# m-schuetz/SimLOD

Hardware: AMD Instinct MI355X
Metric: M points/sec inserted into octree (raster M samples/s @1080p under 'raster') (higher is better)
Workload: dtype f32+u32 (fp32 quantise/project, fp64 pixel coordinate, integer octree/atomics); 1 GPU; Morro Bay 36M stand-in (BASELINE config 2): 36000000 16 B points, fractal terrain, 36 x 1M ring batches resident in HBM, reset + 2.0 kernel_construct launches per step; raster 1920x1080; points_per_gpu=36000000, record_order=shuffled, parallelism=one global cube, level-3 cells dealt to 1 rank(s) by point count

## Files before the change

simlod_amd/csrc/construct.hip:

```cpp
#include <mutex>
#include "simlod_device.hpp"
#include "simlod_hip.h"
#include "simlod_internal.hpp"

namespace simlod {
namespace build {

#include "construct_state.inc"
#include "construct_begin.inc"
#include "construct_count.inc"
#include "construct_expand.inc"
#include "construct_voxelize.inc"
#include "construct_insert.inc"

static_assert(offsetof(Ctl, groupMax) == 44 && offsetof(Ctl, expandNs) + 4 * sizeof(uint64_t) == 184, "Ctl.groupMax at byte 44, Ctl.expandNs[4] at byte 184");

static inline uint64_t align_up(uint64_t v, uint64_t a) { return (v + a - 1) / a * a; }

static constexpr uint64_t ACCT_SPILL_FLOOR = 3500000;
bool layout_construct(BuildArgs& a, uint64_t capacity, bool coalesce, uint32_t groupLimit = SIMLOD_MAX_BATCHES_PER_LAUNCH, uint32_t exactGroup = 1) {
	a.dirCap = 2 * a.nodeCapacity + 65536;
	a.acct = exactGroup > 1u ? 1u : 0u;
	uint64_t off = 4096;
	a.offQueue = off;    off += align_up((uint64_t)CHUNK_QUEUE_CAPACITY * 8, 256);
	a.offSlots = off;    off += align_up((uint64_t)2 * SLOT_CAP * sizeof(SlotRec), 256);
	a.offHist = off;     off += align_up(((uint64_t)SLOT_CAP * HIST_BINS + HIST_EXTRA_WORDS) * 4, 256);
	a.offMap = off;      off += align_up((uint64_t)SLOT_CAP * HIST_BINS * 4, 256);
	a.offHistB = off;    off += align_up((uint64_t)(a.acct ? SLOT_CAP : 0u) * HIST_BINS * exactGroup * 4, 256);
	a.clearCap = 65536;
	a.offClear = off;    off += align_up((uint64_t)2 * a.clearCap * 8, 256);
	a.offTouched = off;  off += align_up((uint64_t)a.nodeCapacity * 4, 256);
	a.crossCap = 16384;
	a.offCross = off;    off += align_up((uint64_t)a.crossCap * 4, 256);
	a.offSplitTag = off; off += align_up((uint64_t)a.nodeCapacity * 8, 256);
	a.offRetryTag = off; off += align_up((uint64_t)a.nodeCapacity * 4, 256);
	a.offTouchTag = off; off += align_up((uint64_t)a.nodeCapacity * 4, 256);
	a.offStartOf = off;  off += align_up((uint64_t)a.nodeCapacity * 8, 256);
	a.offCntB = off;     off += align_up((uint64_t)(a.acct ? a.nodeCapacity : 0u) * exactGroup * 4, 256);
	a.hashCap = 1u << 17;
	a.offHashDir = off;  off += align_up((uint64_t)a.hashCap * sizeof(DirEntry), 256);
	a.offParent = off;   off += align_up((uint64_t)a.nodeCapacity * 4, 256);
	a.offNodeDir = off;  off += align_up((uint64_t)a.nodeCapacity * sizeof(NodeDir), 256);
	a.offChunkDir = off; off += align_up(2ull * a.dirCap * 8, 256);
	a.offLeafChunks = off; off += (uint64_t)a.nodeCapacity * LEAF_ROW_BYTES;
	a.offPaths = off; off += align_up((uint64_t)a.nodeCapacity * PATH_ROW * 8, 256);
	a.offTop = off;   off += align_up((uint64_t)TOP_CELLS * 4, 256);
	a.offKid = off;   off += align_up((uint64_t)a.nodeCapacity * 4, 256);
	a.voxItemCap = min(a.nodeCapacity + 2u * VOX_BIG_ITEMS, 1u << 20);
	a.offVoxItems = off; off += align_up(2ull * a.voxItemCap * sizeof(VoxItem), 256);
	const uint64_t perBatch = (uint64_t)SIMLOD_MAX_BATCH_SIZE * 4;
	const uint64_t fixedWork = ((uint64_t)SPILLING_CAPACITY + a.nodeCapacity / 8) * 32;
	a.groupMax = 1; a.groupCap = SIMLOD_MAX_BATCH_SIZE;
	if (capacity < off + 2 * perBatch + fixedWork + 4096 + 25ull * 65536) { a.spilledCap = 0; a.scratchBytes = off + 2 * perBatch + fixedWork; return false; }
	const uint64_t freeBytes = capacity - off - fixedWork - 4096;
	if (coalesce) a.groupMax = (uint32_t)std::max<uint64_t>(1, std::min<uint64_t>(std::min<uint32_t>(groupLimit, SIMLOD_MAX_BATCHES_PER_LAUNCH), freeBytes / (2 * perBatch + 20ull * SIMLOD_MAX_BATCH_SIZE)));
	if (a.acct) {
		if (freeBytes < 2ull * exactGroup * perBatch + 512 + ACCT_SPILL_FLOOR * 20032 / 1000) return false;
		a.groupMax = exactGroup;
	}
	a.groupCap = a.groupMax * SIMLOD_MAX_BATCH_SIZE;
	uint64_t cap = (freeBytes - 2ull * a.groupMax * perBatch - 512) * 1000 / (20 * 1000 + 32);
	if (cap > 0x7fffffffull - a.groupCap) cap = 0x7fffffffull - a.groupCap;
	a.spilledCap = (uint32_t)cap;
	a.workCap = a.spilledCap / SIMLOD_POINTS_PER_CHUNK + a.nodeCapacity / 8 + SPILLING_CAPACITY;
	a.offWork = off;     off += align_up((uint64_t)a.workCap * 32, 256);
	a.leafOfStride = align_up((uint64_t)a.groupCap * 4, 256) / 4;
	a.offLeafOf = off;   off += 2 * a.leafOfStride * 4 + align_up((uint64_t)a.spilledCap * 4, 256);
	a.offSpilled = off;  off += (uint64_t)a.spilledCap * 16;
	a.scratchBytes = off;
	return off <= capacity;
}

}
struct SideStream {
	hipStream_t stream;
	hipEvent_t expanded[SIMLOD_MAX_BATCHES_PER_LAUNCH], inserted[SIMLOD_MAX_BATCHES_PER_LAUNCH], tailDone;
	std::mutex enqueue;
};
void destroy_side_stream(SideStream* s) {
	(void)hipStreamSynchronize(s->stream);
	for (uint32_t i = 0; i < SIMLOD_MAX_BATCHES_PER_LAUNCH; i++) { (void)hipEventDestroy(s->expanded[i]); (void)hipEventDestroy(s->inserted[i]); }
	(void)hipEventDestroy(s->tailDone);
	(void)hipStreamDestroy(s->stream);
	delete s;
}
namespace build {
#ifndef SYNC_EVENT_FLAGS
#define SYNC_EVENT_FLAGS (hipEventDisableTiming | hipEventDisableSystemFence)
#endif
static SideStream* side_stream(Context& ctx) {
	int dev = 0;
	(void)hipGetDevice(&dev);
	if (dev < 0 || dev >= 64) return nullptr;
	std::lock_guard<std::mutex> hold(ctx.sideLock);
	if (ctx.side[dev] == nullptr) {
		SideStream* s = new SideStream();
		bool ok = hipStreamCreateWithFlags(&s->stream, hipStreamNonBlocking) == hipSuccess;
		const unsigned flags = ctx.tune(KNOB_EVENT_SYSTEM_FENCE, 0) != 0 ? (unsigned)hipEventDisableTiming : (unsigned)SYNC_EVENT_FLAGS;
		for (uint32_t i = 0; ok && i < SIMLOD_MAX_BATCHES_PER_LAUNCH; i++)
			ok = hipEventCreateWithFlags(&s->expanded[i], flags) == hipSuccess && hipEventCreateWithFlags(&s->inserted[i], flags) == hipSuccess;
		ok = ok && hipEventCreateWithFlags(&s->tailDone, flags) == hipSuccess;
		if (!ok) { (void)hipGetLastError(); delete s; return nullptr; }
		ctx.side[dev] = s;
	}
	return ctx.side[dev];
}

int launch_construct(Context& ctx, const SimlodUniforms* u, SimlodPoint* points, uint32_t* buffer, uint8_t* pers, SimlodNode* nodes,
                     SimlodStats* stats, uint64_t* frameStart, uint32_t* numBatchesUploaded, uint32_t* batchSizes, hipStream_t stream) {
	BuildArgs a{};
	a.ring = points; a.mom = reinterpret_cast<uint8_t*>(buffer); a.pers = pers; a.nodes = nodes; a.stats = stats;
	a.frameStart = frameStart; a.numBatchesUploaded = numBatchesUploaded; a.batchSizes = batchSizes;
	octree_box(u, a.size, a.minx, a.miny, a.minz);
	a.persCapacity = u->persistentBufferCapacity;
	a.frameCounter = u->frameCounter;
	a.nodeCapacity = ctx.nodeCapacity.load();
	a.trunkLo = ctx.trunkLo.load(); a.trunkHi = ctx.trunkHi.load();
	const bool coalesce = ctx.ingestMode.load() != 0u;
	uint32_t exactGroup = coalesce || ctx.tune(KNOB_DEBUG_BUDGET_US, 0) > 0 ? 1u : (uint32_t)std::min<int>(std::max(1, ctx.tune(KNOB_EXACT_GROUP, 5)), (int)ACCT_MAX_GROUP);
	if (exactGroup > 1u && SIMLOD_MEM_SAFETY_MARGIN + group_slack_bytes(2ull * SIMLOD_MAX_BATCH_SIZE, 0u) >= a.persCapacity) exactGroup = 1u;
	bool fits = false;
	for (; exactGroup > 1u && !fits; exactGroup -= fits ? 0u : 1u) fits = layout_construct(a, u->momentaryBufferCapacity, false, 1, exactGroup);
	if (!fits) fits = layout_construct(a, u->momentaryBufferCapacity, coalesce, (uint32_t)std::max(1, ctx.tune(KNOB_GROUP_BATCHES, 10)));
	if (fits && ((uint64_t)a.mom & (LEAF_ROW_BYTES - 1u)) == 0ull) {
		const Ctl* ctl = reinterpret_cast<const Ctl*>(a.mom);
		note_leaf_table(ctx, LeafTableRef{nodes, a.mom, a.mom + a.offLeafChunks, a.pers, &ctl->tableMagic, &ctl->tableBatch,
		                             &ctl->tableNodes, &ctl->tableSig, TABLE_MAGIC, LEAF_SLOTS, a.nodeCapacity});
	} else forget_leaf_table(ctx, nodes);
	const DeviceInfo& dev = device_info();

	note_upload_counter(numBatchesUploaded, 0u, false, true);
	const LaunchPlan plan = launch_plan(ctx, nodes, numBatchesUploaded);
	const uint32_t limit = plan.batches;
	const uint32_t take = a.acct != 0u && !plan.mayGroup ? 1u : a.groupMax;
	SIMLOD_LAUNCH(k_begin, dim3(fits ? dev.numCUs * 2 : 1u), dim3(TPB), stream, a, fits ? 0u : 1u, limit, ((uint32_t)ctx.tune(KNOB_DEBUG_FORCE_BARRIER_TIMEOUT, 0) & 1u) | (ctx.tune(KNOB_DEBUG_VOXELIZE_CLOCK, 0) != 0 ? 2u : 0u) | (plan.sideTablesStale ? 4u : 0u) | (ctx.tune(KNOB_DEBUG_IRREGULAR_CHILDREN, 0) != 0 ? 8u : 0u) | (((uint32_t)ctx.tune(KNOB_DEBUG_PHASE_WG, 0) & 0xffffu) << 8),
	              (uint32_t)std::max(0, ctx.tune(KNOB_DEBUG_BUDGET_US, 0)), take);
	if (fits) {
		const uint32_t gridPoints = dev.numCUs * (uint32_t)ctx.tune(KNOB_GRID_MULT, 8);
		const uint32_t numGroups = (limit + take - 1u) / take;
		const bool overlap = ctx.tune(KNOB_OVERLAP_TAIL, 1) != 0 && !profile_enabled() && numGroups > 1u;
		const bool single = take == 1u || limit <= 1u;
		const uint32_t expandWgs = (uint32_t)max(1, min(ctx.tune(KNOB_EXPAND_WGS, !single ? (int)dev.numCUs / 2 : (int)dev.numCUs / (overlap ? 4 : 2)), (int)dev.numCUs));
		SideStream* side = overlap ? side_stream(ctx) : nullptr;
		std::unique_lock<std::mutex> block;
		if (side != nullptr) block = std::unique_lock<std::mutex>(side->enqueue);
		const int countTpb = ctx.tune(KNOB_COUNT_TPB, 512);
		hipStream_t back = side != nullptr ? side->stream : stream;
		auto fail = [&](hipError_t e) { if (side != nullptr) (void)hipStreamSynchronize(side->stream); (void)hipGetLastError(); return (int)(e != hipSuccess ? e : hipErrorUnknown); };
		const uint32_t voxWgs = (uint32_t)max(1, ctx.tune(KNOB_VOXELIZE_WGS, (int)dev.numCUs * 2)) + VOXROOT_WGS;
		for (uint32_t b = 0; b < numGroups; b++) {
			if (single) {
				if (countTpb == 256) SIMLOD_LAUNCH((k_count<TPB, true>), dim3(gridPoints), dim3(TPB), stream, a, b);
				else SIMLOD_LAUNCH((k_count<512, true>), dim3(gridPoints / 2), dim3(512), stream, a, b);
			} else SIMLOD_LAUNCH((k_count<512, false>), dim3(gridPoints / 2), dim3(512), stream, a, b);
			SIMLOD_LAUNCH(k_queue, dim3(single ? 16 : 128), dim3(TPB), stream, a, b);
			if (side != nullptr && b > 0) { const hipError_t e = hipStreamWaitEvent(stream, side->inserted[b - 1], 0); if (e != hipSuccess) return fail(e); }
			SIMLOD_LAUNCH(k_hist, dim3(gridPoints), dim3(TPB), stream, a, b);
			if (!single) {
				SIMLOD_LAUNCH(k_expand<true>, dim3(expandWgs), dim3(ETPB), stream, a, b, 0u, 1u);
				SIMLOD_LAUNCH(k_hist2, dim3(gridPoints), dim3(TPB), stream, a, b);
			}
			const hipEvent_t expanded = side != nullptr ? side->expanded[b] : nullptr, inserted = side != nullptr ? side->inserted[b] : nullptr;
			const bool gated = expand_gate_enter(ctx, stream);
			SIMLOD_LAUNCH_STOP(k_expand<false>, dim3(expandWgs), dim3(ETPB), stream, expanded, a, b, single ? 0u : 1u, (uint32_t)SIMLOD_MAX_EXPAND_ROUNDS);
			expand_gate_leave(ctx, stream, expanded, gated);
			if (side != nullptr) { const hipError_t e = hipStreamWaitEvent(back, expanded, 0); if (e != hipSuccess) return fail(e); }
			if (!single && a.acct != 0u) SIMLOD_LAUNCH(k_rootpre, dim3(1), dim3(1024), back, a, b);
			if (single) SIMLOD_LAUNCH_STOP(k_insert<true>, dim3(gridPoints), dim3(TPB), back, inserted, a, b);
			else SIMLOD_LAUNCH_STOP(k_insert<false>, dim3(gridPoints), dim3(TPB), back, inserted, a, b);
			if (profile_dominant()) {
				hipEvent_t e0, e1;
				profile_kernel_events("k_voxelize", &e0, &e1);
				hipExtLaunchKernelGGL(k_voxelize, dim3(voxWgs), dim3(VTPB), 0, back, e0, e1, 0, a, b);
				{ const hipError_t e = hipGetLastError(); if (e != hipSuccess) return fail(e); }
			} else
			SIMLOD_LAUNCH(k_voxelize, dim3(voxWgs), dim3(VTPB), back, a, b);
		}
		if (side != nullptr) {
			hipError_t e = hipEventRecord(side->tailDone, back);
			if (e == hipSuccess) e = hipStreamWaitEvent(stream, side->tailDone, 0);
			if (e != hipSuccess) return fail(e);
		}
		const uint32_t gridNodes = (a.nodeCapacity + TPB - 1) / TPB;
		SIMLOD_LAUNCH(k_voxdone, dim3(min(gridNodes, dev.numCUs)), dim3(TPB), stream, a);
		SIMLOD_LAUNCH(k_stats, dim3(min(gridNodes, dev.numCUs)), dim3(TPB), stream, a);
	}
	SIMLOD_LAUNCH(k_finish, dim3(1), dim3(64), stream, a, fits ? 1u : 0u, plan.feedback, (const uint32_t*)numBatchesUploaded, plan.seq);
	if (profile_enabled()) profile_close(stream);
	hipError_t e = hipGetLastError();
	if (e != hipSuccess) return (int)e;
	return fits ? 0 : (int)hipErrorInvalidValue;
}

uint64_t construct_min_bytes(uint32_t nodeCapacity) {
	BuildArgs a{};
	a.nodeCapacity = nodeCapacity;
	layout_construct(a, 0, false);
	return a.scratchBytes + 4096 + 26ull * 65536;
}

}
}
```

simlod_amd/csrc/construct_expand.inc:

```

static constexpr uint32_t VTPB = 1024;
#ifndef VOX_SPT_N
#define VOX_SPT_N 8
#endif
static constexpr uint32_t VOX_SPT = VOX_SPT_N;
static constexpr uint32_t VOX_PIECE = VTPB * VOX_SPT;
static constexpr uint32_t VOX_BIG_ITEMS = 65536;
static constexpr uint32_t VOX_SMALL = 512;
static constexpr uint32_t VOX_SMALL_PIECE = 128;
static constexpr uint32_t LDS_LEVELS = 7;
static constexpr uint32_t CUBE_WORDS = 8192 + 1024 + 256 + 64 + 16 + 4 + 4;
struct VoxItem { uint32_t leaf, s0, s1, ptBase, ptFirst; };
__device__ __forceinline__ VoxItem* vox_items(const BuildArgs& a, const BatchCtl* bc) { return at<VoxItem>(a, a.offVoxItems) + (uint64_t)(bc->ordinal & 1u) * a.voxItemCap; }

#ifndef ALLOC_WAVES_N
#define ALLOC_WAVES_N 10
#endif
static constexpr uint32_t ALLOC_WAVES = ALLOC_WAVES_N, ALLOC_LEAVES = 64 * ALLOC_WAVES;
struct AllocRec {
	uint32_t node, existing, additional, fromPool;
	uint32_t dirNew, prefix;
	unsigned long long firstIdx, mem;
	SimlodChunk* head; SimlodChunk* tail;
};
// ... 65 lines not shown
		dirBase = (uint32_t)__shfl((int)dirBase, 0, 64); itemBase = (uint32_t)__shfl((int)itemBase, 0, 64); smallBase = (uint32_t)__shfl((int)smallBase, 0, 64);
		chunkBase = shfl64(chunkBase, 0);
		const unsigned long long firstIdx = chunkBase + exAdditional;
		const uint32_t fromPool = firstIdx >= pool ? 0u : (uint32_t)min((unsigned long long)additional, pool - firstIdx);
		uint32_t totNew;
		const uint32_t exNew = wave_exclusive(additional - fromPool, totNew);
		unsigned long long mem = 0;
		if (lane == 0u && totNew != 0u) mem = (unsigned long long)persistent_alloc(a.pers, sizeof(SimlodChunk), totNew);
		mem = shfl64(mem, 0) + (unsigned long long)exNew * SIMLOD_ALLOC_ROUND(sizeof(SimlodChunk));
		const uint32_t base = dirBase + exEntries;
		const uint32_t itemAt = pieces != 0u ? itemBase + exPieces : VOX_BIG_ITEMS + smallBase + exSmall;
		bool ok = need;
		if (need && base + entries > a.dirCap) { panic(ctl, SIMLOD_ERR_DIRECTORY_FULL); ok = false; }
		if (need && (pieces != 0u ? itemAt + pieces > VOX_BIG_ITEMS : itemAt + small > a.voxItemCap)) { panic(ctl, SIMLOD_ERR_DIRECTORY_FULL); ok = false; }
		uint32_t e = 0;
		if (ok) {
			if (first < existing) chunkDir[base + e++] = tail;
			NodeDir& d = nodeDir[i];
			d.ptBase = base; d.ptFirst = first; d.ptTag = bc->tag;
			VoxItem* items = vox_items(a, bc);
			const uint32_t nl = fresh_leaves ? fl.level : node->level;
			if (pieces == 0u) for (uint32_t q = 0; q < small; q++) items[itemAt + q] = VoxItem{i | nl << 24, stored + q * VOX_SMALL_PIECE, min(stored + (q + 1u) * VOX_SMALL_PIECE, counter), base, first};
			else for (uint32_t q = 0; q < pieces; q++) items[itemAt + q] = VoxItem{i | nl << 24, stored + q * VOX_PIECE, min(stored + (q + 1u) * VOX_PIECE, counter), base, first};
		}
		AllocRec& r = rec[threadIdx.x];
		r.node = i; r.existing = existing; r.additional = ok ? additional : 0u; r.fromPool = fromPool; r.dirNew = base + e; r.prefix = exAdditional;
		r.firstIdx = firstIdx; r.mem = mem; r.head = head; r.tail = tail;
	}
	__syncthreads();
	uint32_t total = 0;
	for (uint32_t w = 0; w < waves; w++) total += sh.waveTotal[w];
	for (uint32_t q0 = threadIdx.x; q0 < total; q0 += blockDim.x) {
		uint32_t q = q0, wv = 0;
		while (wv + 1u < waves && q >= sh.waveTotal[wv]) { q -= sh.waveTotal[wv]; wv++; }
		uint32_t lo = wv * 64u, hi = lo + 64u;
		while (hi - lo > 1u) { const uint32_t mid = (lo + hi) >> 1; if (rec[mid].prefix <= q) lo = mid; else hi = mid; }
		const AllocRec r = rec[lo];
		const uint32_t k = q - r.prefix;
		if (k >= r.additional) continue;
		auto chunk_at = [&](uint32_t j) -> SimlodChunk* {
			return j < r.fromPool ? chunkQueue[r.firstIdx + j] : reinterpret_cast<SimlodChunk*>(r.mem + (unsigned long long)(j - r.fromPool) * SIMLOD_ALLOC_ROUND(sizeof(SimlodChunk)));
		};
		SimlodChunk* c = chunk_at(k);
		SimlodChunk* next = k + 1u < r.additional ? chunk_at(k + 1u) : nullptr;
		SimlodChunk* first = r.head != nullptr ? r.head : (k == 0u ? c : (k + 1u == r.additional ? chunk_at(0u) : nullptr));
		c->next = next;
		chunkDir[r.dirNew + k] = c;
		if (r.existing + k < LEAF_SLOTS) leaf_row_set(leafChunks, a.pers, r.node, r.existing + k, c);
		if (k == 0u) { if (r.tail == nullptr) a.nodes[r.node].points = c; else r.tail->next = c; }
		if (k + 1u == r.additional) tail_of(first) = c;
	}
}

__global__ __launch_bounds__(TPB) void k_hist(BuildArgs a, uint32_t ordinal) {
	Ctl* ctl = ctl_of(a);
	BatchCtl* bc = batch_of(ctl, ordinal);
	if (bc == nullptr || ctl->abortBatch) return;
	const uint32_t n = bc->batchSize, tag = bc->tag, numWork = bc->numWork;
	const uint32_t slots0 = slots_in_use(bc);
	if (blockIdx.x == 0 && threadIdx.x == 0) bc->slotsRound0 = slots0;
	if (blockIdx.x + 1u == gridDim.x && threadIdx.x == 0) prepare_batch(a, ctl, ordinal + 1u);
	if (slots0 == 0u) return;
	__shared__ BlockTable tbl;
	const LeafWords leafOf(a, ordinal);
	const unsigned long long* slotOf = at<const unsigned long long>(a, a.offSplitTag);
	uint32_t* hist = at<uint32_t>(a, a.offHist);
	const uint32_t shard = blockIdx.x & (HIST_SHARDS - 1u);
	const SpillWork* work = at<const SpillWork>(a, a.offWork);
	float4* spilled = at<float4>(a, a.offSpilled);
	const uint32_t moved = min(numWork, a.workCap) * SIMLOD_POINTS_PER_CHUNK;
	const uint32_t total = moved + n;
	const uint32_t numChunks = (total + CPB - 1) / CPB;
	if (blockIdx.x >= numChunks) return;
	Phase ph(ctl, blockIdx.x == 0);
	table_init(tbl);
	__syncthreads();
	const bool acct = bc->acct != 0u;
	uint32_t* histB = at<uint32_t>(a, a.offHistB);
	const uint32_t GB = a.groupMax;
	auto flush = [&](uint32_t key, uint32_t cnt) {
		const uint32_t kb = key >> ACCT_BATCH_SHIFT, k21 = key & 0x1fffffu;
		if (acct && kb != ACCT_MOVED) atomicAdd(histB + (uint64_t)k21 * GB + kb, cnt);
		else atomicAdd(hist + hist_word(k21, shard), cnt);
	};
	auto add = [&](uint32_t key, uint32_t kb) {
		uint32_t rank;
		if (acct) key |= kb << ACCT_BATCH_SHIFT;
		if (table_add(tbl, key, 1u, &rank) < 0) flush(key, 1u);
	};
	const Samples<false> grp(a, bc);
	for (uint32_t chunk = blockIdx.x; chunk < numChunks; chunk += gridDim.x) {
		const float4* unusedBase; uint32_t kspan = 0;
		const uint32_t e0 = max(chunk * CPB, moved), e1 = min(total, (chunk + 1u) * CPB);
		const bool oneBatch = acct && e0 < e1 && grp.span(e0 - moved, e1 - 1u - moved, unusedBase, kspan);
		uint32_t ent[HCPT], dst[HCPT], v[HCPT];
		const float4* src[HCPT];
#pragma unroll
		for (uint32_t j = 0; j < HCPT; j++) {
			const uint32_t e = chunk * CPB + j * TPB + threadIdx.x;
			ent[j] = NONE; src[j] = nullptr; dst[j] = 0; v[j] = NONE;
			if (e < moved) {
				const SpillWork item = work[e / SIMLOD_POINTS_PER_CHUNK];
				const uint32_t k = e % SIMLOD_POINTS_PER_CHUNK;
				if (k < item.count) { ent[j] = (item.level << 16) | item.slot; src[j] = reinterpret_cast<const float4*>(item.chunk->points) + k; dst[j] = item.dstBase + k; }
			} else if (e < total) v[j] = leafOf.grp[e - moved];
		}
		unsigned long long info[HCPT];
#pragma unroll
		for (uint32_t j = 0; j < HCPT; j++) info[j] = v[j] != NONE ? slotOf[v[j] & LEAF_NODE_MASK] : 0ull;
		float4 p[HCPT];
#pragma unroll
		for (uint32_t j = 0; j < HCPT; j++) p[j] = ent[j] != NONE ? *src[j] : make_float4(0, 0, 0, 0);
#pragma unroll
		for (uint32_t j = 0; j < HCPT; j++) {
			if (v[j] == NONE || (uint32_t)(info[j] >> 32) != tag) continue;
			const uint32_t key = (((uint32_t)info[j] & 0xffffu) << 9) | (v[j] >> LEAF_BIN_SHIFT);
			const uint32_t i = chunk * CPB + j * TPB + threadIdx.x - moved;
			leafOf.grp[i] = LEAF_FLAG | key;
			add(key, !acct ? 0u : oneBatch ? kspan : batch_of_sample(bc, i));
		}
#pragma unroll
		for (uint32_t j = 0; j < HCPT; j++) {
			if (ent[j] == NONE) continue;
			const uint32_t X = quantize(F_GRID, p[j].x, a.minx, a.size), Y = quantize(F_GRID, p[j].y, a.miny, a.size), Z = quantize(F_GRID, p[j].z, a.minz, a.size);
			const uint32_t key = ((ent[j] & 0xffffu) << 9) | bin_of(X, Y, Z, ent[j] >> 16);
			spilled[dst[j]] = p[j]; leafOf.mov[dst[j]] = LEAF_FLAG | key;
			add(key, ACCT_MOVED);
		}
	}
	__syncthreads();
	ph.mark(4);
	for (uint32_t e = threadIdx.x; e < (uint32_t)TBL_CAP; e += TPB) {
		const uint32_t key = tbl.keys[e];
		if (key != TBL_EMPTY) flush(key, tbl.vals[e]);
	}
	ph.mark(5);
	if (ph.on) ctl->phaseNs[6] += 1;
}

static constexpr uint32_t ETPB = 1024;
static constexpr int HT_BITS = 12;
static constexpr uint32_t HT_CAP = 1u << HT_BITS;
static constexpr uint32_t LOCAL_NODES = 8 + 64 + 512;

__device__ __forceinline__ uint32_t hist_sum(const uint32_t* hist, uint64_t word) {
	uint32_t v = hist[word];
	if ((word >> 9) < HIST_SHARDED) {
#pragma unroll
		for (uint32_t sd = 1; sd < HIST_SHARDS; sd++) v += hist[hist_word((uint32_t)word, sd)];
	}
	return v;
}

__device__ __forceinline__ uint32_t bin_total(const BuildArgs& a, const uint32_t* hist, uint64_t word, bool acct) {
	uint32_t v = hist_sum(hist, word);
	if (acct) {
		const uint32_t* hb = at<const uint32_t>(a, a.offHistB) + word * a.groupMax;
		for (uint32_t k = 0; k < a.groupMax; k++) v += hb[k];
	}
	return v;
}
static constexpr uint32_t ACCT_MAX_GROUP = 12;
static constexpr uint32_t NEVER = 0xffu;

struct ExpandShared {
	union {
		struct { uint32_t keys[HT_CAP], vals[HT_CAP]; };
		AllocRec allocRec[ALLOC_LEAVES];
	};
	uint32_t bins[HIST_BINS], c2[64], c1[8];
	uint32_t base2[8], base3[64];
	uint32_t listed[LOCAL_NODES];
	FreshLeaf fresh[LOCAL_NODES];
	uint32_t LX, LY, LZ;
	uint8_t nameL[20];
	SimlodOccupancyGrid* gridL;
	uint32_t numFresh, numFill;
	uint32_t part[ETPB / 64u];
	uint32_t nextGranted, nextSlot, nextChild, clearBase;
	uint8_t* gridMem;
	uint32_t fillStart[LOCAL_NODES];
	uint4 fill[LOCAL_NODES];
	AllocShared alloc;
	SimlodOccupancyGrid* grid[8 + 64];
	unsigned long long pathL[PATH_WORDS];
	uint32_t mask1, extraBase, ok, more;
	unsigned long long mask2;
	uint8_t splitAt[LOCAL_NODES + 8];
	uint32_t counterAt[LOCAL_NODES + 1];
	uint32_t forced1;
	unsigned long long forced2;
// ... 533 lines not shown
```

simlod_amd/csrc/construct_insert.inc:

```


__device__ void voxdone_nodes(const BuildArgs& a, Ctl* ctl, uint32_t tag, uint32_t numNodes, uint32_t first, uint32_t stride, bool skipRoot = false) {
	for (uint32_t i = first; i < numNodes; i += stride) {
		if (skipRoot && i == 0u) continue;
		SimlodNode* node = a.nodes + i;
		const uint32_t numVoxels = node->numVoxels, stored = node->numVoxelsStored;
		if (numVoxels == stored) continue;
		const uint32_t existing = (stored + SIMLOD_POINTS_PER_CHUNK - 1) / SIMLOD_POINTS_PER_CHUNK, last = (numVoxels - 1u) / SIMLOD_POINTS_PER_CHUNK;
		if (last >= existing) {
			SimlodChunk* tail = dir_find(a, tag, i, last);
			if (tail != nullptr) { tail->next = nullptr; tail_of(node->voxelChunks) = tail; } else raise(ctl, SIMLOD_ERR_NULL_CHUNK);
		}
		node->numVoxelsStored = numVoxels;
	}
}
__global__ __launch_bounds__(TPB) void k_voxdone(BuildArgs a) {
	Ctl* ctl = ctl_of(a);
	if (ctl->processed == 0u || ctl->abortBatch) return;
	voxdone_nodes(a, ctl, ctl->tagOf[ctl->processed - 1u], min(a.stats->numNodes, a.nodeCapacity), blockIdx.x * TPB + threadIdx.x, gridDim.x * TPB);
}

__global__ __launch_bounds__(1024) void k_rootpre(BuildArgs a, uint32_t ordinal) {
	Ctl* ctl = ctl_of(a);
	BatchCtl* bc = batch_of(ctl, ordinal);
	if (bc == nullptr || ctl->abortBatch || bc->acct == 0u) return;
	const uint32_t sR = bc->rootSplitAt;
	if (sR == NONE || sR == 0u) return;
	if (threadIdx.x == 0u && ordinal > 0u) voxdone_nodes(a, ctl, ctl->tagOf[ordinal - 1u], 1u, 0u, 1u);
	__threadfence();
	__syncthreads();
	const uint32_t n = bc->start[min(sR, bc->groupBatches)], lane = (uint32_t)lane_id();
	const Samples<false> pts(a, bc);
	SimlodOccupancyGrid* const g = a.nodes[0].grid;
	if (g == nullptr) return;
	for (uint32_t base = 0; base < n; base += blockDim.x) {
		const uint32_t i = base + threadIdx.x;
		bool go = i < n;
		const float4 p = go ? pts[i] : make_float4(0, 0, 0, 0);
		const uint32_t pX = quantize(F_FULL, p.x, a.minx, a.size), pY = quantize(F_FULL, p.y, a.miny, a.size), pZ = quantize(F_FULL, p.z, a.minz, a.size);
		const uint32_t cell = grid_cell(0u, pX, pY, pZ), bit = cell & 31u;
		uint32_t* word = &g->values[cell >> 5];
		go = go && ((*word >> bit) & 1u) == 0u;
		go = go && ((atomicOr(word, go ? 1u << bit : 0u) >> bit) & 1u) == 0u;
		const unsigned long long wm = __ballot(go);
		if (wm == 0ull) continue;
		uint32_t first = 0;
		if (lane == 0u) first = atomicAdd(&a.nodes[0].numVoxels, (uint32_t)__popcll(wm));
		first = (uint32_t)__shfl((int)first, 0, 64);
		store_voxels_wave(a, ctl, bc->tag, go, 0u, first + (uint32_t)__popcll(wm & ((1ull << lane) - 1ull)), voxel_of(a, 0, pX, pY, pZ, p.w));
	}
}

struct InsertShared {
	BlockTable tbl;
	uint32_t base[TBL_CAP];
	uint32_t dirBase[TBL_CAP];
	uint32_t dirFirst[TBL_CAP];
};

template <bool SINGLE>
__global__ __launch_bounds__(TPB) void k_insert(BuildArgs a, uint32_t ordinal) {
	Ctl* ctl = ctl_of(a);
	BatchCtl* bc = batch_of(ctl, ordinal);
	if (bc == nullptr) return;
	if (ctl->abortBatch) {
		if (blockIdx.x == 0 && threadIdx.x == 0) end_of_batch(a, ctl, bc);
		return;
	}
	__shared__ InsertShared sh;
	const uint32_t n = bc->batchSize;
	const uint32_t total = n + min(bc->numSpilled, a.spilledCap);
	const Samples<SINGLE> pts(a, bc);
	const float4* spilled = at<const float4>(a, a.offSpilled);
	const LeafWords leafOf(a, ordinal);
	const NodeDir* nodeDir = at<const NodeDir>(a, a.offNodeDir);
// ... 157 lines not shown
```

simlod_amd/csrc/simlod_hip.cpp:

```cpp
#include <dlfcn.h>

#include <atomic>
#include <cstdio>
#include <cstdlib>
#include <cstring>
#include <mutex>
#include <string>
#include <utility>
#include <vector>

#include "simlod_hip.h"
#include "simlod_internal.hpp"

namespace simlod {

const char* const KNOB_NAMES[KNOB_COUNT_] = {
	"SIMLOD_OVERLAP_TAIL", "SIMLOD_EXPAND_WGS", "SIMLOD_GRID_MULT", "SIMLOD_COUNT_TPB", "SIMLOD_VOXELIZE_WGS", "SIMLOD_ADAPTIVE_GROUPS",
	"SIMLOD_RASTER_LEAF_TABLE", "SIMLOD_RASTER_LDS_TILES", "SIMLOD_DRAW_MULT", "SIMLOD_RASTER_FUSED_RESOLVE",
	"SIMLOD_DEBUG_FORCE_BARRIER_TIMEOUT", "SIMLOD_DEBUG_VOXELIZE_CLOCK", "SIMLOD_DEBUG_BUDGET_US", "SIMLOD_GROUP_BATCHES", "SIMLOD_DEBUG_PHASE_WG", "SIMLOD_EVENT_SYSTEM_FENCE", "SIMLOD_RASTER_SCREEN_BINS", "SIMLOD_DEBUG_BIN_POOL", "SIMLOD_EXACT_GROUP", "SIMLOD_DEBUG_IRREGULAR_CHILDREN",
};

static std::atomic<uint32_t> g_liveContexts{0};
uint32_t live_contexts() { return g_liveContexts.load(); }

Context::Context() { reload_env(); g_liveContexts.fetch_add(1); }

namespace {
struct ExpandGate { std::mutex lock; hipEvent_t last = nullptr; const Context* owner = nullptr; };
ExpandGate g_gate[64];
int gate_device() { int dev = 0; (void)hipGetDevice(&dev); return dev < 0 || dev >= 64 ? 0 : dev; }
}

bool expand_gate_enter(Context& ctx, hipStream_t stream) {
	ExpandGate& g = g_gate[gate_device()];
	g.lock.lock();
	if (g.last != nullptr && g.owner != &ctx) (void)hipStreamWaitEvent(stream, g.last, 0);
	return true;
}

void expand_gate_leave(Context& ctx, hipStream_t stream, hipEvent_t ended, bool held) {
	if (!held) return;
	const int dev = gate_device();
	ExpandGate& g = g_gate[dev];
	if (ended == nullptr) {
		if (ctx.gateEvent[dev] == nullptr && hipEventCreateWithFlags(&ctx.gateEvent[dev], hipEventDisableTiming) != hipSuccess) { (void)hipGetLastError(); ctx.gateEvent[dev] = nullptr; }
		ended = ctx.gateEvent[dev];
		if (ended != nullptr) (void)hipEventRecord(ended, stream);
	}
	if (ended != nullptr) { g.last = ended; g.owner = &ctx; }
	g.lock.unlock();
}

void expand_gate_forget(Context& ctx) {
	for (ExpandGate& g : g_gate) {
		std::lock_guard<std::mutex> hold(g.lock);
		if (g.owner == &ctx) { g.last = nullptr; g.owner = nullptr; }
	}
}

void Context::reload_env() {
	for (int k = 0; k < KNOB_COUNT_; k++) {
		const char* v = std::getenv(KNOB_NAMES[k]);
		knob[k] = v != nullptr && *v != 0 ? std::atoi(v) : KNOB_UNSET;
	}
}

Context::~Context() {
	expand_gate_forget(*this);
	g_liveContexts.fetch_sub(1);
	for (SideStream*& s : side) { if (s != nullptr) destroy_side_stream(s); s = nullptr; }
	(void)hipDeviceSynchronize();
	for (OctreeState& o : octrees) (void)hipHostFree(const_cast<uint32_t*>(o.history.seen));
// ... 561 lines not shown
```

simlod_amd/csrc/simlod_internal.hpp:

```cpp
#pragma once

#include <hip/hip_runtime.h>
#include <hip/hip_ext.h>
#include <stddef.h>
#include <stdint.h>

#include <atomic>
#include <climits>
#include <mutex>
#include <vector>

#include "simlod_abi.h"
#include "simlod_hip.h"
#include "octree_state.hpp"

namespace simlod {

static constexpr uint32_t CHUNK_QUEUE_CAPACITY = 1000000u;
static constexpr uint32_t SPILLING_CAPACITY = 100000u;

static constexpr uint32_t LEAF_ROW_SLOTS = SIMLOD_MAX_POINTS_PER_NODE / SIMLOD_POINTS_PER_CHUNK, LEAF_ROW_BYTES = 256;
static_assert(LEAF_ROW_SLOTS * 5u <= LEAF_ROW_BYTES && LEAF_ROW_SLOTS * 4u % 4u == 0u, "leaf chunk table row");
__host__ __device__ inline const SimlodChunk* leaf_row_get(const uint8_t* table, const uint8_t* pers, uint64_t row, uint32_t k) {
	const uint8_t* r = table + row * LEAF_ROW_BYTES;
	const uint64_t v = (uint64_t)reinterpret_cast<const uint32_t*>(r)[k] | (uint64_t)r[LEAF_ROW_SLOTS * 4u + k] << 32;
	return v != 0ull ? reinterpret_cast<const SimlodChunk*>(pers + (v << 4)) : nullptr;
}
__host__ __device__ inline void leaf_row_set(uint8_t* table, const uint8_t* pers, uint64_t row, uint32_t k, const SimlodChunk* c) {
	uint8_t* r = table + row * LEAF_ROW_BYTES;
	const uint64_t v = c != nullptr ? (uint64_t)(reinterpret_cast<const uint8_t*>(c) - pers) >> 4 : 0ull;
	reinterpret_cast<uint32_t*>(r)[k] = (uint32_t)v;
	r[LEAF_ROW_SLOTS * 4u + k] = (uint8_t)(v >> 32);
}
__host__ __device__ inline uint64_t table_signature(const SimlodStats* s) {
	return ((uint64_t)s->numNodes | (uint64_t)s->numPoints << 32) ^ (s->allocatedBytes_persistent * 0x9E3779B97F4A7C15ull) ^ ((uint64_t)s->numVoxels << 20);
}
inline void octree_box(const SimlodUniforms* u, float& size, float& minx, float& miny, float& minz) {
	const float bx = u->boxMax.x - u->boxMin.x, by = u->boxMax.y - u->boxMin.y, bz = u->boxMax.z - u->boxMin.z;
	size = fmaxf(fmaxf(bx, by), bz);
	minx = u->boxMin.x; miny = u->boxMin.y; minz = u->boxMin.z;
}
enum Knob : int {
	KNOB_OVERLAP_TAIL, KNOB_EXPAND_WGS, KNOB_GRID_MULT, KNOB_COUNT_TPB, KNOB_VOXELIZE_WGS, KNOB_ADAPTIVE_GROUPS,
	KNOB_RASTER_LEAF_TABLE, KNOB_RASTER_LDS_TILES, KNOB_DRAW_MULT, KNOB_RASTER_FUSED_RESOLVE,
	KNOB_DEBUG_FORCE_BARRIER_TIMEOUT, KNOB_DEBUG_VOXELIZE_CLOCK, KNOB_DEBUG_BUDGET_US, KNOB_GROUP_BATCHES, KNOB_DEBUG_PHASE_WG, KNOB_EVENT_SYSTEM_FENCE, KNOB_RASTER_SCREEN_BINS, KNOB_DEBUG_BIN_POOL, KNOB_EXACT_GROUP, KNOB_DEBUG_IRREGULAR_CHILDREN, KNOB_COUNT_
};
static constexpr int KNOB_UNSET = INT_MIN;
extern const char* const KNOB_NAMES[KNOB_COUNT_];

struct FrameFeedback { const void* buffer; volatile uint32_t* seen; bool bins; uint64_t bytes; bool possible, open; };
struct SideStream;
void destroy_side_stream(SideStream* s);

struct ArrayState { bool rendered, imported; };

struct Context {
	std::atomic<uint32_t> nodeCapacity{263157u};
	std::atomic<uint32_t> ingestMode{0u};
	std::atomic<uint32_t> batchLimit{SIMLOD_MAX_BATCHES_PER_LAUNCH};
	std::atomic<int>      hintPending{-1};
	std::atomic<uint64_t> trunkLo{0u}, trunkHi{0u};
	int knob[KNOB_COUNT_];
	std::mutex sideLock;
	SideStream* side[64] = {};
	std::mutex octreesLock;
	std::vector<OctreeState> octrees;
	std::mutex framesLock;
	std::vector<FrameFeedback> frames;
	hipEvent_t gateEvent[64] = {};
	Context();
	~Context();
	void reload_env();
	int tune(Knob k, int dflt) const { return knob[k] == KNOB_UNSET ? dflt : knob[k]; }
};
uint32_t* frame_feedback(Context& ctx, const void* buffer, uint32_t parts, bool& possible, bool& bins, uint64_t& bufferBytes);
void frame_feedback_no_bins(Context& ctx, const void* buffer);
void array_event(Context& ctx, const void* nodes, ArrayEvent e);
ArrayState array_state(Context& ctx, const void* nodes);
Context& context_of(const void* nodes);
uint32_t live_contexts();

bool expand_gate_enter(Context& ctx, hipStream_t stream);
void expand_gate_leave(Context& ctx, hipStream_t stream, hipEvent_t ended, bool held);
void expand_gate_forget(Context& ctx);

namespace build {

int launch_construct(Context& ctx, const SimlodUniforms* u, SimlodPoint* points, uint32_t* buffer, uint8_t* pers, SimlodNode* nodes,
                     SimlodStats* stats, uint64_t* frameStart, uint32_t* numBatchesUploaded, uint32_t* batchSizes, hipStream_t stream);
uint64_t construct_min_bytes(uint32_t nodeCapacity);

}

void note_leaf_table(Context& ctx, const LeafTableRef& ref);
void forget_leaf_table(Context& ctx, const void* nodes);
void octree_image_replaced(Context& ctx, const void* nodes);
bool find_leaf_table(Context& ctx, const void* nodes, LeafTableRef& ref);

// ... 65 lines not shown
```

Before: 15640 M points/s.

## Split histogram into samples/moved passes and overlap with side-stream voxelize

```diff
diff --git a/simlod_amd/csrc/construct.hip b/simlod_amd/csrc/construct.hip
--- a/simlod_amd/csrc/construct.hip
+++ b/simlod_amd/csrc/construct.hip
@@ -1,7 +1,9 @@
 #include <mutex>
+#include <vector>
 #include "simlod_device.hpp"
 #include "simlod_hip.h"
 #include "simlod_internal.hpp"
+#include "launch_chain.hpp"
 
 namespace simlod {
 namespace build {
@@ -75,11 +77,12 @@
 struct SideStream {
 	hipStream_t stream;
 	hipEvent_t expanded[SIMLOD_MAX_BATCHES_PER_LAUNCH], inserted[SIMLOD_MAX_BATCHES_PER_LAUNCH], tailDone;
+	hipEvent_t queued[SIMLOD_MAX_BATCHES_PER_LAUNCH], moved[SIMLOD_MAX_BATCHES_PER_LAUNCH];
 	std::mutex enqueue;
 };
 void destroy_side_stream(SideStream* s) {
 	(void)hipStreamSynchronize(s->stream);
-	for (uint32_t i = 0; i < SIMLOD_MAX_BATCHES_PER_LAUNCH; i++) { (void)hipEventDestroy(s->expanded[i]); (void)hipEventDestroy(s->inserted[i]); }
+	for (uint32_t i = 0; i < SIMLOD_MAX_BATCHES_PER_LAUNCH; i++) { (void)hipEventDestroy(s->expanded[i]); (void)hipEventDestroy(s->inserted[i]); (void)hipEventDestroy(s->queued[i]); (void)hipEventDestroy(s->moved[i]); }
 	(void)hipEventDestroy(s->tailDone);
 	(void)hipStreamDestroy(s->stream);
 	delete s;
@@ -98,7 +101,8 @@
 		bool ok = hipStreamCreateWithFlags(&s->stream, hipStreamNonBlocking) == hipSuccess;
 		const unsigned flags = ctx.tune(KNOB_EVENT_SYSTEM_FENCE, 0) != 0 ? (unsigned)hipEventDisableTiming : (unsigned)SYNC_EVENT_FLAGS;
 		for (uint32_t i = 0; ok && i < SIMLOD_MAX_BATCHES_PER_LAUNCH; i++)
-			ok = hipEventCreateWithFlags(&s->expanded[i], flags) == hipSuccess && hipEventCreateWithFlags(&s->inserted[i], flags) == hipSuccess;
+			ok = hipEventCreateWithFlags(&s->expanded[i], flags) == hipSuccess && hipEventCreateWithFlags(&s->inserted[i], flags) == hipSuccess &&
+			     hipEventCreateWithFlags(&s->queued[i], flags) == hipSuccess && hipEventCreateWithFlags(&s->moved[i], flags) == hipSuccess;
 		ok = ok && hipEventCreateWithFlags(&s->tailDone, flags) == hipSuccess;
 		if (!ok) { (void)hipGetLastError(); delete s; return nullptr; }
 		ctx.side[dev] = s;
@@ -148,38 +152,63 @@
 		hipStream_t back = side != nullptr ? side->stream : stream;
 		auto fail = [&](hipError_t e) { if (side != nullptr) (void)hipStreamSynchronize(side->stream); (void)hipGetLastError(); return (int)(e != hipSuccess ? e : hipErrorUnknown); };
 		const uint32_t voxWgs = (uint32_t)max(1, ctx.tune(KNOB_VOXELIZE_WGS, (int)dev.numCUs * 2)) + VOXROOT_WGS;
-		for (uint32_t b = 0; b < numGroups; b++) {
-			if (single) {
-				if (countTpb == 256) SIMLOD_LAUNCH((k_count<TPB, true>), dim3(gridPoints), dim3(TPB), stream, a, b);
-				else SIMLOD_LAUNCH((k_count<512, true>), dim3(gridPoints / 2), dim3(512), stream, a, b);
-			} else SIMLOD_LAUNCH((k_count<512, false>), dim3(gridPoints / 2), dim3(512), stream, a, b);
-			SIMLOD_LAUNCH(k_queue, dim3(single ? 16 : 128), dim3(TPB), stream, a, b);
-			if (side != nullptr && b > 0) { const hipError_t e = hipStreamWaitEvent(stream, side->inserted[b - 1], 0); if (e != hipSuccess) return fail(e); }
-			SIMLOD_LAUNCH(k_hist, dim3(gridPoints), dim3(TPB), stream, a, b);
-			if (!single) {
-				SIMLOD_LAUNCH(k_expand<true>, dim3(expandWgs), dim3(ETPB), stream, a, b, 0u, 1u);
-				SIMLOD_LAUNCH(k_hist2, dim3(gridPoints), dim3(TPB), stream, a, b);
+		auto event_of = [&](const ChainStep& st) -> hipEvent_t {
+			if (side == nullptr) return nullptr;
+			switch (st.event) {
+				case EV_QUEUED: return side->queued[st.group];
+				case EV_MOVED: return side->moved[st.group];
+				case EV_EXPANDED: return side->expanded[st.group];
+				case EV_INSERTED: return side->inserted[st.group];
+				default: return nullptr;
 			}
-			const hipEvent_t expanded = side != nullptr ? side->expanded[b] : nullptr, inserted = side != nullptr ? side->inserted[b] : nullptr;
-			const bool gated = expand_gate_enter(ctx, stream);
-			SIMLOD_LAUNCH_STOP(k_expand<false>, dim3(expandWgs), dim3(ETPB), stream, expanded, a, b, single ? 0u : 1u, (uint32_t)SIMLOD_MAX_EXPAND_ROUNDS);
-			expand_gate_leave(ctx, stream, expanded, gated);
-			if (side != nullptr) { const hipError_t e = hipStreamWaitEvent(back, expanded, 0); if (e != hipSuccess) return fail(e); }
-			if (!single && a.acct != 0u) SIMLOD_LAUNCH(k_rootpre, dim3(1), dim3(1024), back, a, b);
-			if (single) SIMLOD_LAUNCH_STOP(k_insert<true>, dim3(gridPoints), dim3(TPB), back, inserted, a, b);
-			else SIMLOD_LAUNCH_STOP(k_insert<false>, dim3(gridPoints), dim3(TPB), back, inserted, a, b);
-			if (profile_dominant()) {
-				hipEvent_t e0, e1;
-				profile_kernel_events("k_voxelize", &e0, &e1);
-				hipExtLaunchKernelGGL(k_voxelize, dim3(voxWgs), dim3(VTPB), 0, back, e0, e1, 0, a, b);
-				{ const hipError_t e = hipGetLastError(); if (e != hipSuccess) return fail(e); }
-			} else
-			SIMLOD_LAUNCH(k_voxelize, dim3(voxWgs), dim3(VTPB), back, a, b);
-		}
-		if (side != nullptr) {
-			hipError_t e = hipEventRecord(side->tailDone, back);
-			if (e == hipSuccess) e = hipStreamWaitEvent(stream, side->tailDone, 0);
-			if (e != hipSuccess) return fail(e);
+		};
+		std::vector<ChainStep> steps;
+		chain_steps(steps, numGroups, side != nullptr, ctx.tune(KNOB_HIST_SPLIT, 1), !single, !single && a.acct != 0u);
+		for (const ChainStep& st : steps) {
+			const uint32_t b = st.group;
+			const hipStream_t on = st.back != 0 ? back : stream;
+			const hipEvent_t ev = event_of(st);
+			switch (st.op) {
+			case OP_COUNT:
+				if (single) {
+					if (countTpb == 256) SIMLOD_LAUNCH((k_count<TPB, true>), dim3(gridPoints), dim3(TPB), on, a, b);
+					else SIMLOD_LAUNCH((k_count<512, true>), dim3(gridPoints / 2), dim3(512), on, a, b);
+				} else SIMLOD_LAUNCH((k_count<512, false>), dim3(gridPoints / 2), dim3(512), on, a, b);
+				break;
+			case OP_QUEUE:
+				SIMLOD_LAUNCH_STOP(k_queue, dim3(single ? 16 : 128), dim3(TPB), on, ev, a, b);
+				break;
+			case OP_WAIT: { const hipError_t e = hipStreamWaitEvent(on, ev, 0); if (e != hipSuccess) return fail(e); } break;
+			case OP_HIST: SIMLOD_LAUNCH(k_hist, dim3(gridPoints), dim3(TPB), on, a, b); break;
+			case OP_HIST_SAMPLES: SIMLOD_LAUNCH(k_hist_samples, dim3(gridPoints), dim3(TPB), on, a, b); break;
+			case OP_HIST_MOVED: SIMLOD_LAUNCH_STOP(k_hist_moved, dim3(max(1u, gridPoints / 4u)), dim3(TPB), on, ev, a, b); break;
+			case OP_EXPAND_ROUND0: SIMLOD_LAUNCH(k_expand<true>, dim3(expandWgs), dim3(ETPB), on, a, b, 0u, 1u); break;
+			case OP_HIST2: SIMLOD_LAUNCH(k_hist2, dim3(gridPoints), dim3(TPB), on, a, b); break;
+			case OP_EXPAND: {
+				const bool gated = expand_gate_enter(ctx, on);
+				SIMLOD_LAUNCH_STOP(k_expand<false>, dim3(expandWgs), dim3(ETPB), on, ev, a, b, single ? 0u : 1u, (uint32_t)SIMLOD_MAX_EXPAND_ROUNDS);
+				expand_gate_leave(ctx, on, ev, gated);
+			} break;
+			case OP_ROOTPRE: SIMLOD_LAUNCH(k_rootpre, dim3(1), dim3(ROOTPRE_TPB), on, a, b); break;
+			case OP_INSERT:
+				if (single) SIMLOD_LAUNCH_STOP(k_insert<true>, dim3(gridPoints), dim3(TPB), on, ev, a, b);
+				else SIMLOD_LAUNCH_STOP(k_insert<false>, dim3(gridPoints), dim3(TPB), on, ev, a, b);
+				break;
+			case OP_VOXELIZE:
+				if (profile_dominant()) {
+					hipEvent_t e0, e1;
+					profile_kernel_events("k_voxelize", &e0, &e1);
+					hipExtLaunchKernelGGL(k_voxelize, dim3(voxWgs), dim3(VTPB), 0, on, e0, e1, 0, a, b);
+					{ const hipError_t e = hipGetLastError(); if (e != hipSuccess) return fail(e); }
+				} else
+				SIMLOD_LAUNCH(k_voxelize, dim3(voxWgs), dim3(VTPB), on, a, b);
+				break;
+			case OP_TAIL: {
+				hipError_t e = hipEventRecord(side->tailDone, back);
+				if (e == hipSuccess) e = hipStreamWaitEvent(stream, side->tailDone, 0);
+				if (e != hipSuccess) return fail(e);
+			} break;
+			}
 		}
 		const uint32_t gridNodes = (a.nodeCapacity + TPB - 1) / TPB;
 		SIMLOD_LAUNCH(k_voxdone, dim3(min(gridNodes, dev.numCUs)), dim3(TPB), stream, a);
diff --git a/simlod_amd/csrc/construct_expand.inc b/simlod_amd/csrc/construct_expand.inc
--- a/simlod_amd/csrc/construct_expand.inc
+++ b/simlod_amd/csrc/construct_expand.inc
@@ -141,14 +141,18 @@
 	}
 }
 
-__global__ __launch_bounds__(TPB) void k_hist(BuildArgs a, uint32_t ordinal) {
+static constexpr uint32_t HIST_SAMPLES = 1u, HIST_MOVED = 2u, HIST_BOTH = 3u;
+template <uint32_t PARTS>
+__device__ __forceinline__ void hist_pass(const BuildArgs& a, uint32_t ordinal) {
 	Ctl* ctl = ctl_of(a);
 	BatchCtl* bc = batch_of(ctl, ordinal);
 	if (bc == nullptr || ctl->abortBatch) return;
-	const uint32_t n = bc->batchSize, tag = bc->tag, numWork = bc->numWork;
+	const uint32_t n = bc->batchSize, tag = bc->tag, numWork = (PARTS & HIST_MOVED) != 0u ? bc->numWork : 0u;
 	const uint32_t slots0 = slots_in_use(bc);
-	if (blockIdx.x == 0 && threadIdx.x == 0) bc->slotsRound0 = slots0;
-	if (blockIdx.x + 1u == gridDim.x && threadIdx.x == 0) prepare_batch(a, ctl, ordinal + 1u);
+	if ((PARTS & HIST_MOVED) != 0u) {
+		if (blockIdx.x == 0 && threadIdx.x == 0) bc->slotsRound0 = slots0;
+		if (blockIdx.x + 1u == gridDim.x && threadIdx.x == 0) prepare_batch(a, ctl, ordinal + 1u);
+	}
 	if (slots0 == 0u) return;
 	__shared__ BlockTable tbl;
 	const LeafWords leafOf(a, ordinal);
@@ -158,7 +162,7 @@
 	const SpillWork* work = at<const SpillWork>(a, a.offWork);
 	float4* spilled = at<float4>(a, a.offSpilled);
 	const uint32_t moved = min(numWork, a.workCap) * SIMLOD_POINTS_PER_CHUNK;
-	const uint32_t total = moved + n;
+	const uint32_t total = (PARTS & HIST_SAMPLES) != 0u ? moved + n : moved;
 	const uint32_t numChunks = (total + CPB - 1) / CPB;
 	if (blockIdx.x >= numChunks) return;
 	Phase ph(ctl, blockIdx.x == 0);
@@ -188,11 +192,11 @@
 		for (uint32_t j = 0; j < HCPT; j++) {
 			const uint32_t e = chunk * CPB + j * TPB + threadIdx.x;
 			ent[j] = NONE; src[j] = nullptr; dst[j] = 0; v[j] = NONE;
-			if (e < moved) {
+			if ((PARTS & HIST_MOVED) != 0u && e < moved) {
 				const SpillWork item = work[e / SIMLOD_POINTS_PER_CHUNK];
 				const uint32_t k = e % SIMLOD_POINTS_PER_CHUNK;
 				if (k < item.count) { ent[j] = (item.level << 16) | item.slot; src[j] = reinterpret_cast<const float4*>(item.chunk->points) + k; dst[j] = item.dstBase + k; }
-			} else if (e < total) v[j] = leafOf.grp[e - moved];
+			} else if ((PARTS & HIST_SAMPLES) != 0u && e < total) v[j] = leafOf.grp[e - moved];
 		}
 		unsigned long long info[HCPT];
 #pragma unroll
@@ -226,6 +230,9 @@
 	ph.mark(5);
 	if (ph.on) ctl->phaseNs[6] += 1;
 }
+__global__ __launch_bounds__(TPB) void k_hist(BuildArgs a, uint32_t ordinal) { hist_pass<HIST_BOTH>(a, ordinal); }
+__global__ __launch_bounds__(TPB) void k_hist_samples(BuildArgs a, uint32_t ordinal) { hist_pass<HIST_SAMPLES>(a, ordinal); }
+__global__ __launch_bounds__(TPB) void k_hist_moved(BuildArgs a, uint32_t ordinal) { hist_pass<HIST_MOVED>(a, ordinal); }
 
 static constexpr uint32_t ETPB = 1024;
 static constexpr int HT_BITS = 12;
diff --git a/simlod_amd/csrc/construct_insert.inc b/simlod_amd/csrc/construct_insert.inc
--- a/simlod_amd/csrc/construct_insert.inc
+++ b/simlod_amd/csrc/construct_insert.inc
@@ -20,7 +20,11 @@
 	voxdone_nodes(a, ctl, ctl->tagOf[ctl->processed - 1u], min(a.stats->numNodes, a.nodeCapacity), blockIdx.x * TPB + threadIdx.x, gridDim.x * TPB);
 }
 
-__global__ __launch_bounds__(1024) void k_rootpre(BuildArgs a, uint32_t ordinal) {
+#ifndef ROOTPRE_TPB_N
+#define ROOTPRE_TPB_N 256
+#endif
+static constexpr uint32_t ROOTPRE_TPB = ROOTPRE_TPB_N;
+__global__ __launch_bounds__(ROOTPRE_TPB) void k_rootpre(BuildArgs a, uint32_t ordinal) {
 	Ctl* ctl = ctl_of(a);
 	BatchCtl* bc = batch_of(ctl, ordinal);
 	if (bc == nullptr || ctl->abortBatch || bc->acct == 0u) return;
diff --git a/simlod_amd/csrc/launch_chain.hpp b/simlod_amd/csrc/launch_chain.hpp
--- /dev/null
+++ b/simlod_amd/csrc/launch_chain.hpp
@@ -0,0 +1,46 @@
+#pragma once
+#include <stdint.h>
+#include <vector>
+
+namespace simlod {
+enum ChainOp : uint8_t {
+	OP_COUNT, OP_QUEUE, OP_HIST, OP_HIST_SAMPLES, OP_HIST_MOVED, OP_EXPAND_ROUND0, OP_HIST2, OP_EXPAND, OP_ROOTPRE, OP_INSERT, OP_VOXELIZE,
+	OP_WAIT,
+	OP_TAIL
+};
+enum ChainEvent : uint8_t { EV_NONE, EV_QUEUED, EV_MOVED, EV_EXPANDED, EV_INSERTED };
+struct ChainStep { uint8_t op, back, event; uint32_t group; };
+
+inline int chain_mode(bool twoStreams, int histSplit) { return twoStreams && (histSplit == 1 || histSplit == 2) ? histSplit : 0; }
+inline void chain_steps(std::vector<ChainStep>& out, uint32_t numGroups, bool twoStreams, int histSplit, bool grouped, bool rootpre) {
+	const int mode = chain_mode(twoStreams, histSplit);
+	auto push = [&](ChainOp op, bool back, uint32_t b, ChainEvent ev = EV_NONE) { out.push_back(ChainStep{(uint8_t)op, (uint8_t)(back ? 1 : 0), (uint8_t)ev, b}); };
+	out.clear();
+	for (uint32_t b = 0; b < numGroups; b++) {
+		push(OP_COUNT, false, b);
+		push(OP_QUEUE, false, b, mode == 1 ? EV_QUEUED : EV_NONE);
+		if (mode == 0) {
+			if (twoStreams && b > 0u) push(OP_WAIT, false, b - 1u, EV_INSERTED);
+			push(OP_HIST, false, b);
+		} else if (mode == 2) {
+			push(OP_HIST_SAMPLES, false, b);
+			if (b > 0u) push(OP_WAIT, false, b - 1u, EV_INSERTED);
+			push(OP_HIST_MOVED, false, b);
+		} else {
+			push(OP_HIST_SAMPLES, false, b);
+			push(OP_WAIT, true, b, EV_QUEUED);
+			push(OP_HIST_MOVED, true, b, EV_MOVED);
+			if (b > 0u) push(OP_VOXELIZE, true, b - 1u);
+			push(OP_WAIT, false, b, EV_MOVED);
+		}
+		if (grouped) { push(OP_EXPAND_ROUND0, false, b); push(OP_HIST2, false, b); }
+		push(OP_EXPAND, false, b, twoStreams ? EV_EXPANDED : EV_NONE);
+		if (twoStreams) push(OP_WAIT, true, b, EV_EXPANDED);
+		if (rootpre) push(OP_ROOTPRE, true, b);
+		push(OP_INSERT, true, b, twoStreams && mode != 1 ? EV_INSERTED : EV_NONE);
+		if (mode != 1) push(OP_VOXELIZE, true, b);
+	}
+	if (mode == 1 && numGroups > 0u) push(OP_VOXELIZE, true, numGroups - 1u);
+	if (twoStreams) push(OP_TAIL, false, numGroups);
+}
+}
diff --git a/simlod_amd/csrc/simlod_hip.cpp b/simlod_amd/csrc/simlod_hip.cpp
--- a/simlod_amd/csrc/simlod_hip.cpp
+++ b/simlod_amd/csrc/simlod_hip.cpp
@@ -17,7 +17,7 @@
 const char* const KNOB_NAMES[KNOB_COUNT_] = {
 	"SIMLOD_OVERLAP_TAIL", "SIMLOD_EXPAND_WGS", "SIMLOD_GRID_MULT", "SIMLOD_COUNT_TPB", "SIMLOD_VOXELIZE_WGS", "SIMLOD_ADAPTIVE_GROUPS",
 	"SIMLOD_RASTER_LEAF_TABLE", "SIMLOD_RASTER_LDS_TILES", "SIMLOD_DRAW_MULT", "SIMLOD_RASTER_FUSED_RESOLVE",
-	"SIMLOD_DEBUG_FORCE_BARRIER_TIMEOUT", "SIMLOD_DEBUG_VOXELIZE_CLOCK", "SIMLOD_DEBUG_BUDGET_US", "SIMLOD_GROUP_BATCHES", "SIMLOD_DEBUG_PHASE_WG", "SIMLOD_EVENT_SYSTEM_FENCE", "SIMLOD_RASTER_SCREEN_BINS", "SIMLOD_DEBUG_BIN_POOL", "SIMLOD_EXACT_GROUP", "SIMLOD_DEBUG_IRREGULAR_CHILDREN",
+	"SIMLOD_DEBUG_FORCE_BARRIER_TIMEOUT", "SIMLOD_DEBUG_VOXELIZE_CLOCK", "SIMLOD_DEBUG_BUDGET_US", "SIMLOD_GROUP_BATCHES", "SIMLOD_DEBUG_PHASE_WG", "SIMLOD_EVENT_SYSTEM_FENCE", "SIMLOD_RASTER_SCREEN_BINS", "SIMLOD_DEBUG_BIN_POOL", "SIMLOD_EXACT_GROUP", "SIMLOD_DEBUG_IRREGULAR_CHILDREN", "SIMLOD_HIST_SPLIT",
 };
 
 static std::atomic<uint32_t> g_liveContexts{0};
diff --git a/simlod_amd/csrc/simlod_internal.hpp b/simlod_amd/csrc/simlod_internal.hpp
--- a/simlod_amd/csrc/simlod_internal.hpp
+++ b/simlod_amd/csrc/simlod_internal.hpp
@@ -43,7 +43,7 @@
 enum Knob : int {
 	KNOB_OVERLAP_TAIL, KNOB_EXPAND_WGS, KNOB_GRID_MULT, KNOB_COUNT_TPB, KNOB_VOXELIZE_WGS, KNOB_ADAPTIVE_GROUPS,
 	KNOB_RASTER_LEAF_TABLE, KNOB_RASTER_LDS_TILES, KNOB_DRAW_MULT, KNOB_RASTER_FUSED_RESOLVE,
-	KNOB_DEBUG_FORCE_BARRIER_TIMEOUT, KNOB_DEBUG_VOXELIZE_CLOCK, KNOB_DEBUG_BUDGET_US, KNOB_GROUP_BATCHES, KNOB_DEBUG_PHASE_WG, KNOB_EVENT_SYSTEM_FENCE, KNOB_RASTER_SCREEN_BINS, KNOB_DEBUG_BIN_POOL, KNOB_EXACT_GROUP, KNOB_DEBUG_IRREGULAR_CHILDREN, KNOB_COUNT_
+	KNOB_DEBUG_FORCE_BARRIER_TIMEOUT, KNOB_DEBUG_VOXELIZE_CLOCK, KNOB_DEBUG_BUDGET_US, KNOB_GROUP_BATCHES, KNOB_DEBUG_PHASE_WG, KNOB_EVENT_SYSTEM_FENCE, KNOB_RASTER_SCREEN_BINS, KNOB_DEBUG_BIN_POOL, KNOB_EXACT_GROUP, KNOB_DEBUG_IRREGULAR_CHILDREN, KNOB_HIST_SPLIT, KNOB_COUNT_
 };
 static constexpr int KNOB_UNSET = INT_MIN;
 extern const char* const KNOB_NAMES[KNOB_COUNT_];
```

Measured after the change: 15340 M points/s. 0.98x the previous value.
